# vaultah/replicat

Hardware: AMD Instinct MI355X
Metric: GiB/s chunked, device-resident streams (higher is better)
Workload: dtype u8

## Files before the change

### include/replicat_chunker.h

```cpp
#ifndef REPLICAT_CHUNKER_H
#define REPLICAT_CHUNKER_H

#include <stdint.h>

#ifdef __cplusplus
extern "C" {
#endif

#define RC_OK 0
#define RC_ERR_KEY_LENGTH 1
#define RC_ERR_MIN_GT_MAX 2
#define RC_ERR_BAD_KEY 3
#define RC_ERR_ARGUMENT 10
#define RC_ERR_ALIGN 11
#define RC_ERR_HIP 12
#define RC_ERR_OVERFLOW 13
#define RC_ERR_NO_DEVICE 14
#define RC_ERR_DEVICE_FAULT 15

#define RC_COUNT_OVERFLOW (-1)
#define RC_COUNT_FAULT (-3)

#define RC_OPEN 1u
#define RC_PIPELINED 2u
#define RC_PIPELINE_END 4u

typedef struct rc_chunker rc_chunker;

int rc_version(void);

const char *rc_build_id(void);

const char *rc_last_error(void);

int rc_chunker_create(uint64_t min_length, uint64_t max_length, const uint8_t *key,
                      uint64_t key_len, int device, rc_chunker **out);
void rc_chunker_destroy(rc_chunker *ch);

uint64_t rc_chunker_min_length(const rc_chunker *ch);
uint64_t rc_chunker_max_length(const rc_chunker *ch);

int rc_next_cut(rc_chunker *ch, const uint8_t *buffer, uint64_t size, int final,
                uint64_t *out_cut);

uint64_t rc_cut_capacity(const rc_chunker *ch, uint64_t n, const uint64_t *lens,
                         uint64_t *caps );

int rc_chunk_device(rc_chunker *ch, uint64_t n, const uint8_t *const *d_streams,
                    const uint64_t *lens, const uint64_t *last_piece, uint32_t flags,
                    uint64_t *d_cuts, int64_t *d_counts, void *hip_stream);

int rc_chunker_overlap(rc_chunker *ch, uint32_t reserve_cus);
uint32_t rc_chunker_overlap_cus(const rc_chunker *ch);
uint64_t rc_chunker_pipelined_calls(const rc_chunker *ch);

int rc_chunk_wait(rc_chunker *ch, void *hip_stream);

int rc_stream_create(int device, void **out_stream);
void rc_stream_destroy(void *stream);

int rc_chunk_host(rc_chunker *ch, uint64_t n, const uint8_t *const *streams,
                  const uint64_t *lens, const uint64_t *last_piece, uint32_t flags,
                  uint64_t *cuts, int64_t *counts);

int rc_chunker_check(rc_chunker *ch);

int rc_timing_enable(rc_chunker *ch, int enable);
int rc_timing_read_kernels(rc_chunker *ch, double *tile_ms, double *edge_ms, double *chain_ms,
                           uint64_t *calls);
int rc_timing_read(rc_chunker *ch, double *phase_a_ms, double *phase_b_ms, uint64_t *calls);

int rc_fill_splitmix(uint8_t *d_dst, uint64_t nbytes, uint64_t seed, uint64_t stream,
                     void *hip_stream);
int rc_fill_splitmix_streams(uint8_t *d_dst, uint64_t n, uint64_t nbytes, uint64_t slot,
                             uint64_t seed, uint64_t first_stream, uint64_t stream_step,
                             void *hip_stream);
int rc_fill_splitmix_at(uint8_t *d_dst, uint64_t nbytes, uint64_t seed, uint64_t stream,
                        uint64_t word0, void *hip_stream);

int rc_read_probe(const uint8_t *d_src, uint64_t nbytes, uint32_t *d_out, void *hip_stream);
int rc_chunker_read_probe(rc_chunker *ch, const uint8_t *d_src, uint64_t nbytes, uint32_t *d_out,
                          void *hip_stream);

uint64_t rc_keys_needed(uint64_t max_length, uint64_t L, uint64_t P);

uint64_t rc_host_key(const rc_chunker *ch, uint64_t d);

int rc_tile_records(rc_chunker *ch, uint64_t n, const uint8_t *const *d_streams,
                    const uint64_t *lens, const uint64_t *last_piece, uint64_t *keys,
                    uint64_t *js, uint64_t *gmax, uint64_t *ghot, uint64_t cap,
                    uint64_t *n_tiles);
uint32_t rc_group_hot_threshold(const rc_chunker *ch);
uint64_t rc_tile_keys(void);

int rc_tile_schedule(uint64_t n_tiles, uint32_t waves, uint32_t permille, uint32_t chunk,
                     uint32_t dyn_min, uint32_t *ranges, uint64_t cap, uint64_t *n_units);

int rc_tables_key(const uint8_t *key16, uint64_t n, const uint64_t *ds, uint64_t *out,
                  uint32_t *top16);

#ifdef __cplusplus
}
#endif

#endif
```

### replicat_amd/_lib.py

```python
import ctypes
import os
import threading

HERE = os.path.dirname(os.path.abspath(__file__))
LIB_PATH = os.environ.get('RC_LIB_PATH') or os.path.join(HERE, 'libreplicat_chunker.so')

RC_OK = 0
RC_ERR_KEY_LENGTH = 1
RC_ERR_MIN_GT_MAX = 2
RC_ERR_BAD_KEY = 3
RC_ERR_DIGEST_SIZE = 4
RC_ERR_B2_PARAM = 5
RC_ERR_KEY_SIZE = 6
RC_ERR_NONCE_SIZE = 7
RC_ERR_TAG = 8
RC_ERR_DIGEST_BITS = 9
RC_ERR_ARGUMENT = 10
RC_ERR_ALIGN = 11
RC_ERR_HIP = 12
RC_ERR_OVERFLOW = 13
RC_ERR_NO_DEVICE = 14
RC_ERR_DEVICE_FAULT = 15
RC_ERR_CORRUPT = 16
RC_ERR_INDEX_FULL = 17
RC_ERR_PROBE_BOUND = 18
RC_INDEX_ABSENT, RC_INDEX_EXHAUSTED = -1, -2
RC_GC_REFERENCED, RC_GC_DELETE, RC_GC_TAG_MISMATCH, RC_GC_EXHAUSTED = 0, 1, 2, 3
RC_COUNT_OVERFLOW = -1
RC_COUNT_FAULT = -3
RC_OPEN = 1
RC_PIPELINED = 2
RC_PIPELINE_END = 4
RC_DIGEST_SLOT = 64
RC_HASH_BLAKE2B, RC_HASH_SHA2, RC_HASH_SHA3 = 0, 1, 2
RC_CIPHER_NONE, RC_CIPHER_AES_GCM, RC_CIPHER_CHACHA20_POLY1305 = 0, 1, 2
RC_CHUNK_OK, RC_CHUNK_BAD_TAG, RC_CHUNK_CORRUPT = 0, 1, 2
RC_TABLE_OK, RC_TABLE_BAD_TAG, RC_TABLE_NOT_CANONICAL = 0, 1, 2
RC_PARTS_OK, RC_PARTS_NOT_CANONICAL = 0, 2
RC_PART_FIRST, RC_PART_LAST = 1, 2
RC_SNAPSHOT_PART_WORDS = 8
RC_SNAPSHOT_TEXT_DESC_BYTES = 32

_u64, _i64, _u32, _int, _p = ctypes.c_uint64, ctypes.c_int64, ctypes.c_uint32, ctypes.c_int, ctypes.c_void_p
SIGNATURES = {
    'rc_version': (_int, []),
    'rc_build_id': (ctypes.c_char_p, []),
    'rc_last_error': (ctypes.c_char_p, []),
    'rc_chunker_create': (_int, [_u64, _u64, _p, _u64, _int, ctypes.POINTER(_p)]),
    'rc_chunker_destroy': (None, [_p]),
    'rc_chunker_min_length': (_u64, [_p]),
    'rc_chunker_max_length': (_u64, [_p]),
    'rc_next_cut': (_int, [_p, _p, _u64, _int, ctypes.POINTER(_u64)]),
    'rc_cut_capacity': (_u64, [_p, _u64, _p, _p]),
    'rc_chunk_device': (_int, [_p, _u64, _p, _p, _p, _u32, _p, _p, _p]),
    'rc_chunk_host': (_int, [_p, _u64, _p, _p, _p, _u32, _p, _p]),
    'rc_chunker_overlap': (_int, [_p, _u32]),
    'rc_chunker_overlap_cus': (_u32, [_p]),
    'rc_chunker_pipelined_calls': (_u64, [_p]),
    'rc_chunker_check': (_int, [_p]),
    'rc_chunk_wait': (_int, [_p, _p]),
    'rc_stream_create': (_int, [_int, ctypes.POINTER(_p)]),
    'rc_stream_destroy': (None, [_p]),
    'rc_timing_enable': (_int, [_p, _int]),
    'rc_timing_read': (_int, [_p, ctypes.POINTER(ctypes.c_double), ctypes.POINTER(ctypes.c_double),
                              ctypes.POINTER(_u64)]),
    'rc_timing_read_kernels': (_int, [_p, ctypes.POINTER(ctypes.c_double),
                                      ctypes.POINTER(ctypes.c_double),
                                      ctypes.POINTER(ctypes.c_double), ctypes.POINTER(_u64)]),
    'rc_fill_splitmix': (_int, [_p, _u64, _u64, _u64, _p]),
    'rc_fill_splitmix_at': (_int, [_p, _u64, _u64, _u64, _u64, _p]),
    'rc_fill_splitmix_streams': (_int, [_p, _u64, _u64, _u64, _u64, _u64, _u64, _p]),
    'rc_read_probe': (_int, [_p, _u64, _p, _p]),
    'rc_chunker_read_probe': (_int, [_p, _p, _u64, _p, _p]),
    'rc_keys_needed': (_u64, [_u64, _u64, _u64]),
    'rc_host_key': (_u64, [_p, _u64]),
    'rc_tables_key': (_int, [_p, _u64, _p, _p, _p]),
    'rc_tile_records': (_int, [_p, _u64, _p, _p, _p, _p, _p, _p, _p, _u64, ctypes.POINTER(_u64)]),
    'rc_group_hot_threshold': (_u32, [_p]),
    'rc_tile_keys': (_u64, []),
    'rc_tile_schedule': (_int, [_u64, _u32, _u32, _u32, _u32, _p, _u64, ctypes.POINTER(_u64)]),
    'rc_blake2b_create': (_int, [_u32, _int, ctypes.POINTER(_p)]),
    'rc_blake2b_destroy': (None, [_p]),
    'rc_blake2b_digest_size': (_u32, [_p]),
    'rc_blake2b_device': (_int, [_p, _u64, _p, _p, _p, _p]),
    'rc_blake2b_host': (_int, [_p, _u64, _p, _p, _p]),
    'rc_blake2b_chunks': (_int, [_p, _p, _u64, _p, _p, _p, _p, _p, _p]),
    'rc_chunk_digest_host': (_int, [_p, _p, _u64, _p, _p, _p, _u32, _p, _p, _p]),
    'rc_blake2b_state_init': (_int, [_u32, _p, _u32, _p, _u32, _p, _u32, _p]),
    'rc_blake2b_update_device': (_int, [_p, _u64, _p, _p, _p, _p, _p, _p]),
    'rc_blake2b_timing_enable': (_int, [_p, _int]),
    'rc_blake2b_timing_read': (_int, [_p, ctypes.POINTER(ctypes.c_double), ctypes.POINTER(_u64)]),
    'rc_blake2b_derive_chunks': (_int, [_p, _p, _u64, _p, _p, _p, _p, _u32, _p, _p]),
    'rc_sha2_create': (_int, [_u32, _int, ctypes.POINTER(_p)]),
    'rc_sha3_create': (_int, [_u32, _int, ctypes.POINTER(_p)]),
    'rc_sha2_state_init': (_int, [_u32, _p]),
    'rc_sha3_state_init': (_int, [_u32, _p]),
    'rc_hash_destroy': (None, [_p]),
    'rc_hash_digest_size': (_u32, [_p]),
    'rc_hash_algorithm': (_u32, [_p]),
    'rc_hash_device': (_int, [_p, _u64, _p, _p, _p, _p]),
    'rc_hash_host': (_int, [_p, _u64, _p, _p, _p]),
    'rc_hash_chunks': (_int, [_p, _p, _u64, _p, _p, _p, _p, _p, _p]),
    'rc_hash_update_device': (_int, [_p, _u64, _p, _p, _p, _p, _p, _p]),
    'rc_hash_timing_enable': (_int, [_p, _int]),
    'rc_hash_timing_read': (_int, [_p, ctypes.POINTER(ctypes.c_double), ctypes.POINTER(_u64)]),
    'rc_gcm_create': (_int, [_u32, _u32, _int, ctypes.POINTER(_p)]),
    'rc_gcm_destroy': (None, [_p]),
    'rc_gcm_key_bytes': (_u32, [_p]),
    'rc_gcm_nonce_bytes': (_u32, [_p]),
    'rc_gcm_encrypt_device': (_int, [_p, _u64, _p, _p, _p, _p, _p, _p]),
    'rc_gcm_decrypt_device': (_int, [_p, _u64, _p, _p, _p, _p, _p, _p]),
    'rc_gcm_encrypt_host': (_int, [_p, _u64, _p, _p, _p, _p, _p]),
    'rc_gcm_decrypt_host': (_int, [_p, _u64, _p, _p, _p, _p, _p]),
    'rc_gcm_chunks_layout': (_u64, [_p, _p, _u64, _p, _p]),
    'rc_gcm_encrypt_chunks': (_int, [_p, _p, _u64, _p, _p, _p, _p, _p, _p, _p, _p]),
    'rc_gcm_encrypt_chunks_select': (_int, [_p, _p, _u64, _p, _p, _p, _p, _p, _p, _p, _p, _p, _p, _p]),
    'rc_gcm_timing_enable': (_int, [_p, _int]),
    'rc_gcm_timing_read': (_int, [_p, ctypes.POINTER(ctypes.c_double), ctypes.POINTER(_u64)]),
    'rc_chacha_create': (_int, [_int, ctypes.POINTER(_p)]),
    'rc_chacha_destroy': (None, [_p]),
    'rc_chacha_key_bytes': (_u32, [_p]),
    'rc_chacha_nonce_bytes': (_u32, [_p]),
    'rc_chacha_encrypt_device': (_int, [_p, _u64, _p, _p, _p, _p, _p, _p]),
    'rc_chacha_decrypt_device': (_int, [_p, _u64, _p, _p, _p, _p, _p, _p]),
    'rc_chacha_encrypt_host': (_int, [_p, _u64, _p, _p, _p, _p, _p]),
    'rc_chacha_decrypt_host': (_int, [_p, _u64, _p, _p, _p, _p, _p]),
    'rc_chacha_chunks_layout': (_u64, [_p, _p, _u64, _p, _p]),
    'rc_chacha_encrypt_chunks': (_int, [_p, _p, _u64, _p, _p, _p, _p, _p, _p, _p, _p]),
    'rc_chacha_encrypt_chunks_select': (_int, [_p, _p, _u64, _p, _p, _p, _p, _p, _p, _p, _p, _p, _p, _p]),
    'rc_chacha_timing_enable': (_int, [_p, _int]),
    'rc_chacha_timing_read': (_int, [_p, ctypes.POINTER(ctypes.c_double), ctypes.POINTER(_u64)]),
    'rc_poly1305_host': (_int, [_u64, _p, _p, _p, _p]),
    'rc_restore_create': (_int, [_p, _int, _p, _p, ctypes.POINTER(_p)]),
    'rc_restore_destroy': (None, [_p]),
    'rc_restore_overhead': (_u32, [_p]),
    'rc_restore_verify_device': (_int, [_p, _u64, _p, _p, _p, _p, _p, _p]),
    'rc_restore_verify_host': (_int, [_p, _u64, _p, _p, _p, _p, _p]),
    'rc_restore_timing_enable': (_int, [_p, _int]),
    'rc_restore_timing_read': (_int, [_p, ctypes.POINTER(ctypes.c_double), ctypes.POINTER(_u64)]),
    'rc_index_create': (_int, [_u32, _u64, _int, ctypes.POINTER(_p)]),
    'rc_index_destroy': (None, [_p]),
    'rc_index_name_bytes': (_u32, [_p]),
    'rc_index_used': (_u64, [_p]),
    'rc_index_add_host': (_int, [_p, _u64, _p, ctypes.POINTER(_u64)]),
    'rc_index_resolve_chunks': (_int, [_p, _p, _u64, _p, _p, _p, ctypes.POINTER(_u64), _p, _p, _p]),
    'rc_index_reserve': (_int, [_p, _u64]),
    'rc_index_lookup_device': (_int, [_p, _u64, _p, _p, _p]),
    'rc_index_resolve_names_device': (_int, [_p, _u64, _p, ctypes.POINTER(_u64), _p, _p, _p]),
    'rc_gc_create': (_int, [_u32, _u32, _p, _u32, _u64, _int, ctypes.POINTER(_p)]),
    'rc_gc_destroy': (None, [_p]),
    'rc_gc_name_bytes': (_u32, [_p]),
    'rc_gc_used': (_u64, [_p]),
    'rc_gc_capacity': (_u64, [_p]),
    'rc_gc_reference_host': (_int, [_p, _u64, _p]),
    'rc_gc_reference_device': (_int, [_p, _u64, _p]),
    'rc_gc_sweep_device': (_int, [_p, _u64, _p, _p, _u64, _p, _p, _p, _p]),
    'rc_gc_sweep_host': (_int, [_p, _u64, _p, _p, _p, _p, ctypes.POINTER(_u64)]),
    'rc_gc_unreferenced_host': (_int, [_p, _u64, _p, _p, _p, _p, ctypes.POINTER(_u64)]),
    'rc_gc_timing_enable': (_int, [_p, _int]),
    'rc_gc_timing_read': (_int, [_p, ctypes.POINTER(ctypes.c_double), ctypes.POINTER(ctypes.c_double),
                                 ctypes.POINTER(ctypes.c_double), ctypes.POINTER(_u64)]),
    'rc_snapshot_create': (_int, [_u32, _int, _p, _p, _int, ctypes.POINTER(_p)]),
# ... 129 lines not shown
```

### replicat_amd/csrc/gclmul.h

```cpp
#pragma once
#include <stdint.h>

namespace rc {

#ifndef RC_TILE_ITERS
#define RC_TILE_ITERS 16
#endif
constexpr int kTileIters = RC_TILE_ITERS;
constexpr int kTileKeys = 64 * 4 * kTileIters;
constexpr int kWaveSize = 64;
constexpr int kTileWaves = 16;
constexpr int kChainWaves = 4;
#ifndef RC_TILE_GROUPS
#define RC_TILE_GROUPS 4
#endif
constexpr int kTileGroups = RC_TILE_GROUPS;
constexpr int kGroupKeys = kTileKeys / kTileGroups;

constexpr uint32_t kPfBytes = 131072;
constexpr uint32_t kFullOff = kPfBytes;
constexpr uint32_t kFullBytes = 2 * 4 * 256 * 8;
constexpr uint32_t kTileLdsBytes = kPfBytes + kFullBytes;

struct KeyTables {
// ... 2 lines not shown
    uint32_t pf[4][256];
};

struct StreamDesc {
    const uint8_t *const *ptr;
    const uint64_t *len;
    const uint64_t *last;
    const uint64_t *jneed;
    const uint64_t *tile_base;
    const uint64_t *cut_base;
    const uint64_t *cut_cap;
    const uint64_t *seg_base;
    const uint64_t *scratch_base;
    const uint64_t *xtiles;
};

struct TileRecord {
    uint64_t key;
    uint64_t j;
};

struct GroupRecord {
    uint64_t max;
    uint64_t hot[kTileGroups];
    uint64_t pad;
};
static_assert(kTileGroups % 2 == 0 && sizeof(GroupRecord) % 16 == 0, "group record layout");

__host__ __device__ inline uint32_t group_hot_threshold(uint64_t window) {
    if (window < (uint64_t)kTileKeys) return 0;
    const uint64_t below = (10 * 65536 + window - 1) / window;
    return below >= 65536 ? 0u : (uint32_t)(65536 - below);
}

struct ChainParams {
    uint64_t min_length;
    uint64_t max_length;
    uint64_t window;
    uint64_t max_steps;
    uint64_t seg_bytes;
    uint64_t seg_cap;
    uint64_t ext_steps;
    const GroupRecord *grp;
    uint64_t n_tiles;
    uint32_t open;
    uint32_t lean;
    uint32_t lane;
    uint32_t hot;
    const uint64_t *fault;
    uint64_t epoch;
};

constexpr uint32_t kCtrErrWord = 32, kCtrStampWord = 34, kCtrFaultsWord = 36;
constexpr int64_t kCountFault = -3;

struct TileSched {
    uint32_t permille = 0;
    uint32_t chunk = 3;
    uint32_t dyn_min = 0;
    uint32_t group = 64;
};

__host__ __device__ inline uint64_t splitmix64(uint64_t x) {
    uint64_t z = x + 0x9E3779B97F4A7C15ull;
    z = (z ^ (z >> 30)) * 0xBF58476D1CE4E5B9ull;
    z = (z ^ (z >> 27)) * 0x94D049BB133111EBull;
    return z ^ (z >> 31);
}

}

extern "C" {
int rc_launch_tiles(const rc::KeyTables *d_tables, rc::StreamDesc desc, uint64_t n_streams,
                    uint64_t n_tiles, rc::TileRecord *d_records, rc::GroupRecord *d_grp,
                    uint32_t hot, uint32_t *d_xlist, uint32_t *d_ctr, uint64_t epoch,
                    void *stream, void *mid_event, uint32_t cus, void *edge_stream, void *tiled,
                    rc::TileSched sched);
uint64_t rc_tie_list_words(uint64_t n_tiles);
enum : uint32_t { RC_JOIN_WALK_ONLY = 1, RC_JOIN_REPAIR = 2 };
int rc_launch_chain(const rc::KeyTables *d_tables, rc::StreamDesc desc, uint64_t n_streams,
                    rc::ChainParams prm, uint64_t n_segs, const rc::TileRecord *d_records,
                    uint64_t *d_cuts, int64_t *d_counts, uint64_t *d_scratch,
                    uint64_t *d_seg_counts, bool any_multi, uint32_t join, void *stream);
int rc_launch_fill(uint8_t *d_dst, uint64_t nbytes, uint64_t seed, uint64_t stream_id,
                   uint64_t word0, void *stream);
int rc_launch_fill_streams(uint8_t *d_dst, uint64_t n, uint64_t nbytes, uint64_t slot,
                           uint64_t seed, uint64_t id0, uint64_t id_step, void *stream);
int rc_launch_read_probe(const uint8_t *d_src, uint64_t nbytes, uint32_t *d_out, uint32_t block,
                         rc::TileSched sched, void *stream);
}
```

### replicat_amd/csrc/kernels.hip

```cpp
#include <hip/hip_runtime.h>
#include <stdint.h>

#include "capi_internal.h"
#include "gclmul.h"
#include "diag.h"

using namespace rc;

namespace {

typedef uint32_t u32x4 __attribute__((ext_vector_type(4)));
typedef __attribute__((address_space(1))) const u32x4 gu32x4;
typedef __attribute__((address_space(1))) const uint32_t gu32;

constexpr int kStreamAux = RC_DIAG_STREAM_AUX;

__device__ __forceinline__ __amdgpu_buffer_rsrc_t tile_rsrc(const uint8_t *base,
                                                             uint32_t bytes = 0xffffffffu) {
    return __builtin_amdgcn_make_buffer_rsrc(const_cast<uint8_t *>(base), 0, bytes, 0x00020000);
}
__device__ __forceinline__ u32x4 ring_load(__amdgpu_buffer_rsrc_t r, uint32_t lane_off, int it) {
    return __builtin_amdgcn_raw_buffer_load_b128(r, lane_off, it * 1024, kStreamAux);
}

// ... 1289 lines not shown
                                                      uint64_t *__restrict__ cuts,
                                                      int64_t *__restrict__ counts,
                                                      uint64_t *__restrict__ scratch,
                                                      uint64_t *__restrict__ seg_counts,
                                                      uint64_t *__restrict__ seg_rcount) {
    if (call_faulted(prm)) {
        fault_counts(counts, n_streams);
        return;
    }
    stage_chain_tables(tab);
    const uint32_t *pf = s_chain_lds;
    const uint64_t *full = reinterpret_cast<const uint64_t *>(s_chain_lds + 1024);
    const uint64_t *tl = full, *th = full + 1024;
    const uint32_t lane = lane_id();
    const uint32_t lb_a = (lane & 31) * 4, lb_b = lb_a | 0x10000u;
    const uint64_t q = (uint64_t)blockIdx.x * (blockDim.x >> 6) +
                       __builtin_amdgcn_readfirstlane(threadIdx.x >> 6);
    if (q >= n_segs) return;
    const uint64_t s = find_index(d.seg_base, n_streams + 1, q);
    const uint64_t sb = sload(d.seg_base + s), nseg = sload(d.seg_base + s + 1) - sb;
    const uint64_t i = q - sb;
    ChainStream st = chain_stream(d, s);
    RC_DIAG_ONLY(st.diag = st.diag && i == (nseg > 8 ? 7 : 0);)
    const bool direct = nseg == 1;
    uint64_t *out = direct ? cuts + sload(d.cut_base + s) : scratch + sload(d.scratch_base + s) + i * prm.seg_cap;
    const uint64_t cap = direct ? sload(d.cut_cap + s) : prm.seg_cap;
    const uint64_t seg_end = (i + 1) * prm.seg_bytes;
    const uint64_t steps = prm.max_steps == 0 ? 1 : prm.max_steps;

    uint64_t pos = i * prm.seg_bytes, n = 0, ext = 0;
    bool overflow = false, term = false;
    RecCache<R> cache;
    auto emit = [&](uint64_t c) {
        if (n >= cap) {
            overflow = true;
            return;
        }
        if (lane == 0) out[n] = c;
        ++n;
    };
    for (;;) {
        if (pos >= st.L || n >= steps) {
            term = true;
            break;
        }
        if (!direct && pos >= seg_end && ext++ >= prm.ext_steps) break;
        uint64_t c1 = 0, c2 = 0;
        int kind;
        if constexpr (kLean) {
            static_assert(R == 1, "the lean step works on the one-row cache");
            kind = chain_step_small(tl, th, pf, rec, st, prm, cache, pos, lb_a, lb_b, c1, c2);
        } else {
            kind = chain_step<R>(tl, th, pf, rec, st, prm, cache, pos, lb_a, lb_b, c1, c2);
        }
        if (kind == kStepStop) {
            term = true;
            break;
        }
        emit(c1);
        if (kind == kStepTail2) emit(c2);
        if (kind != kStepCut) {
            term = true;
            break;
        }
        if (overflow) break;
        pos = c1;
    }
    if (lane == 0) {
        if (direct) {
            counts[s] = overflow ? -1 : (int64_t)n;
        } else {
            const uint64_t v = overflow ? ~0ull : (n | (term ? (1ull << 63) : 0));
            seg_counts[q] = v;
            seg_rcount[q] = v;
        }
    }
}

constexpr int kLaneFull = 8;
constexpr int kLaneIters = kTileIters / kTileGroups;

constexpr uint32_t kLaneHotMax = 4;

__device__ __forceinline__ void lane_groups(bool live, const GroupRecord &g, uint32_t te,
                                            uint32_t a, uint32_t b, uint32_t t16, uint32_t hot,
                                            uint64_t (&mk)[kTileGroups], uint32_t &sc) {
    sc = 0;
#pragma unroll
    for (int q = 0; q < kTileGroups; ++q) mk[q] = 0;
    if (!live) return;
    const uint32_t tj0 = te * kTileKeys;
    const uint32_t qa = (a - tj0) / kGroupKeys, qb = (b - tj0) / kGroupKeys;
#pragma unroll
    for (int q = 0; q < kTileGroups; ++q) {
        if ((uint32_t)q < qa || (uint32_t)q > qb) continue;
        if (((uint32_t)(g.max >> (16 * q)) & 0xffffu) < t16) continue;
        const uint32_t nh = (uint32_t)__popcll(g.hot[q]);
        if (t16 < hot || nh > kLaneHotMax || nh == 0) sc |= 1u << q;
        else mk[q] = g.hot[q];
    }
}

__device__ __forceinline__ uint32_t top16_of(uint32_t e_lo_word, uint32_t e_hi_word) {
    return ((e_lo_word & 0xffff0000u) ^ (e_hi_word << 16)) >> 16;
}

template <int U>
__device__ __forceinline__ void scan_range(const uint64_t *tl, const uint64_t *th,
                                           const uint8_t *base, uint64_t a, uint64_t b,
                                           uint64_t &bk, uint64_t &bj) {
    const uint64_t lane = lane_id();
    for (uint64_t r = a; r <= b; r += 64 * U) {
        uint2 w[U];
#pragma unroll
        for (int u = 0; u < U; ++u) {
            const uint64_t j = min(r + 64 * u + lane, b);
            w[u].x = ld_u32(base + 4 * j - 4);
            w[u].y = ld_u32(base + 4 * j);
        }
#pragma unroll
        for (int u = 0; u < U; ++u) {
            const uint64_t j = r + 64 * u + lane;
            if (j <= b) take_best(full_key(tl, th, w[u].x, w[u].y), j, bk, bj);
        }
    }
}

template <int kCtrl>
__device__ __forceinline__ uint32_t qperm32(uint32_t v) {
    return (uint32_t)__builtin_amdgcn_mov_dpp((int)v, kCtrl, 0xf, 0xf, true);
}
template <int kCtrl>
__device__ __forceinline__ uint64_t qperm64(uint64_t v) {
    return (uint64_t)qperm32<kCtrl>((uint32_t)(v >> 32)) << 32 | qperm32<kCtrl>((uint32_t)v);
}
__device__ __forceinline__ void quad_best32(uint64_t &k, uint32_t &j) {
    {
        const uint64_t ko = qperm64<0xB1>(k);
        const uint32_t jo = qperm32<0xB1>(j);
        if (ko > k || (ko == k && jo < j)) k = ko, j = jo;
    }
    {
        const uint64_t ko = qperm64<0x4E>(k);
        const uint32_t jo = qperm32<0x4E>(j);
        if (ko > k || (ko == k && jo < j)) k = ko, j = jo;
    }
}

struct QuadIter {
    u32x4 v;
    uint32_t p;
};

__device__ __forceinline__ QuadIter qi_load(const uint8_t *base, uint32_t j4, uint32_t a,
                                            uint32_t b) {
    QuadIter x = {u32x4{0u, 0u, 0u, 0u}, 0u};
    if (j4 <= b && j4 + 3 >= a) {
        x.v = *as_global_x4(base + 4ull * j4);
        x.p = ld_u32(base + 4ull * j4 - (j4 ? 4 : 0));
    }
    return x;
}

__device__ __forceinline__ void qi_eval(const uint32_t *pf, const uint64_t *tl, const uint64_t *th,
                                        const uint8_t *base, const QuadIter &x, uint32_t j4,
                                        uint32_t a, uint32_t b, uint32_t t16, uint64_t &lk,
                                        uint32_t &lj) {
    if (!(j4 <= b && j4 + 3 >= a)) return;
    const uint32_t wd[5] = {x.p, x.v.x, x.v.y, x.v.z, x.v.w};
    uint32_t e[5];
#pragma unroll
    for (int k = 0; k < 5; ++k) e[k] = pfc_entry(pf, wd[k]);
    bool have = false, tie = false;
    uint32_t ct = 0, cj = 0, clo = 0, chi = 0;
#pragma unroll
    for (int k = 0; k < 4; ++k) {
        const uint32_t j = j4 + k, t = top16_of(e[k], e[k + 1]);
        const bool in = j >= a && j <= b && t >= t16;
        const bool take = in && (!have || t > ct);
        tie = take ? false : (tie || (in && t == ct));
        ct = take ? t : ct;
        cj = take ? j : cj;
        clo = take ? wd[k] : clo;
        chi = take ? wd[k + 1] : chi;
        have = have || in;
    }
    if (have) take_best32(full_key(tl, th, clo, chi), cj, lk, lj);
    if (tie) {
#pragma unroll 1
        for (uint32_t k = 0; k < 4; ++k) {
            const uint32_t j = j4 + k;
            if (j >= a && j <= b)
                take_best32(full_key(tl, th, ld_u32(base + 4ull * j - 4), ld_u32(base + 4ull * j)), j, lk, lj);
        }
    }
}

constexpr int kQuadTasks = 4;

template <int F>
__global__ __launch_bounds__(256) void rc_quad_chain_kernel(const KeyTables *__restrict__ tab,
                                                            StreamDesc d, uint64_t n_streams,
                                                            ChainParams prm,
                                                            const TileRecord *__restrict__ rec,
                                                            uint64_t *__restrict__ cuts,
                                                            int64_t *__restrict__ counts) {
    static_assert(F % 4 == 0 && kLaneIters == 4, "a quad lane per record row and per iteration");
    if (call_faulted(prm)) {
        fault_counts(counts, n_streams);
        return;
    }
    stage_chain_tables(tab);
    const uint32_t *pf = s_chain_lds;
    const uint64_t *full = reinterpret_cast<const uint64_t *>(s_chain_lds + 1024);
    const uint64_t *tl = full, *th = full + 1024;
    const uint32_t lane = lane_id(), q = lane & 3u;
    const uint64_t gid = ((uint64_t)blockIdx.x * blockDim.x + threadIdx.x) >> 2;
    if (gid - (lane >> 2) >= n_streams) return;
    const bool mine = gid < n_streams;
    const uint64_t s = mine ? gid : n_streams - 1;
    const GroupRecord *grp = prm.grp;
    const uint8_t *base = d.ptr[s];
    const uint64_t L = d.len[s], P = d.last[s];
    const uint64_t tb0 = d.tile_base[s], nt = d.tile_base[s + 1] - tb0;
    uint64_t *out = cuts + d.cut_base[s];
    const uint64_t cap = d.cut_cap[s];
    const uint32_t jmax = L >= 8 ? (uint32_t)((L - 4) / 4) : 0u;
    const uint32_t minl = (uint32_t)prm.min_length, maxl = (uint32_t)prm.max_length;
    const uint32_t T = (uint32_t)prm.window;
    auto gtile = [&](bool use, uint32_t t) -> uint64_t { return use && t < nt ? tb0 + t : prm.n_tiles; };

    uint64_t pos = 0, n = 0;
    bool walking = mine && L > 0 && prm.max_steps > 0, overflow = false;
    RC_DIAG_ONLY(const bool diag = gid < 16 && q == 0;)
    for (;;) {
        if (!__any(walking)) break;
        RC_LSTAMP(1);
        const uint64_t rem = L - pos;
        const bool far = rem >= 2ull * maxl;
        const bool argmax = (P >= pos && P - pos >= maxl) || far;
        const uint32_t s4 = (uint32_t)(pos >> 2);
        const uint32_t ja = s4 + 1, jb = min(s4 + T, jmax);
        const bool win = walking && argmax && T > 0 && ja <= jb;
        const uint32_t t_lo = (ja + kTileKeys - 1) / kTileKeys, t_hi = (jb + 1) / kTileKeys;
        const uint32_t nf = win && t_hi > t_lo ? t_hi - t_lo : 0u;
        const uint32_t a0 = ja, b0 = min(jb, t_lo * kTileKeys - 1), te0 = ja / kTileKeys;
        const uint32_t a1 = t_hi * kTileKeys, b1 = jb, te1 = t_hi;
        bool live0 = win && ja < t_lo * kTileKeys;
        bool live1 = win && t_hi >= t_lo && jb >= a1;

        TileRecord fr[F / 4];
#pragma unroll
        for (int i = 0; i < F / 4; ++i) {
            const uint32_t t = 4 * i + q;
            fr[i] = rec[gtile(t < nf, t_lo + t)];
        }
        const TileRecord r0 = rec[gtile(live0, te0)], r1 = rec[gtile(live1, te1)];
        const GroupRecord g0 = grp[gtile(live0, te0)], g1 = grp[gtile(live1, te1)];
        const bool spec = live0;
        const uint32_t lc = (s4 & 255u) >> 2, qc = (s4 & (kTileKeys - 1)) / kGroupKeys;
        const uint32_t jqc = (s4 & ~(uint32_t)(kGroupKeys - 1)) + 4 * lc;
        QuadIter x[kQuadTasks];
        x[0] = qi_load(base, jqc + 256 * q, spec ? a0 : 1u, spec ? b0 : 0u);

        uint64_t bk = 0;
        uint32_t bj = ~0u;
#pragma unroll
        for (int i = 0; i < F / 4; ++i)
            if (4 * (uint32_t)i + q < nf && fr[i].key != 0) take_best32(fr[i].key, (uint32_t)fr[i].j, bk, bj);
        quad_best32(bk, bj);
        if (live0 && edge_settled<false>(r0.key, (uint32_t)r0.j, a0, b0, bk, bj)) live0 = false;
        if (live1 && edge_settled<true>(r1.key, (uint32_t)r1.j, a1, b1, bk, bj)) live1 = false;
        uint32_t sc0, sc1;
        RC_LSTAMP(2);
        uint64_t h[kTileGroups], t[kTileGroups];
        lane_groups(live0, g0, te0, a0, b0, (uint32_t)(bk >> 48), prm.hot, h, sc0);
        lane_groups(live1, g1, te1, a1, b1, (uint32_t)(bk >> 48), prm.hot, t, sc1);
        static_assert(kTileGroups == 4, "the task queue below spells out four groups");
        auto any_task = [&]() { return (h[0] | h[1] | h[2] | h[3] | t[0] | t[1] | t[2] | t[3]) != 0; };
        auto task = [&](uint32_t &jq, uint32_t &a, uint32_t &b) {
            int r = -1;
            uint32_t g = 0, l = 0;
#define RC_POP(M, R, Q)                            \
    if (r < 0 && M) {                              \
        l = (uint32_t)__builtin_ctzll(M);          \
        M &= M - 1;                                \
        r = R;                                     \
        g = Q;                                     \
    }
            RC_POP(h[0], 0, 0) RC_POP(h[1], 0, 1) RC_POP(h[2], 0, 2) RC_POP(h[3], 0, 3)
            RC_POP(t[0], 1, 0) RC_POP(t[1], 1, 1) RC_POP(t[2], 1, 2) RC_POP(t[3], 1, 3)
#undef RC_POP
            a = 1, b = 0;
            if (r < 0) return;
            jq = (r ? te1 : te0) * kTileKeys + g * kGroupKeys + 4 * l;
            a = r ? a1 : a0;
            b = r ? b1 : b0;
        };
        bool first = false;
#define RC_FIRST(Q)                                              \
    if (spec && qc == Q && (h[Q] >> lc & 1u)) {                  \
        h[Q] &= ~(1ull << lc);                                   \
        first = true;                                            \
    }
        RC_FIRST(0) RC_FIRST(1) RC_FIRST(2) RC_FIRST(3)
#undef RC_FIRST
        uint32_t jq[kQuadTasks], ra[kQuadTasks], rb[kQuadTasks];
        jq[0] = jqc, ra[0] = first ? a0 : 1u, rb[0] = first ? b0 : 0u;
        for (;;) {
            if (!__any(first || any_task())) break;
            bool used[kQuadTasks];
#pragma unroll
            for (int k = 0; k < kQuadTasks; ++k) {
                if (!(k == 0 && first)) {
                    task(jq[k], ra[k], rb[k]);
                    x[k] = qi_load(base, jq[k] + 256 * q, ra[k], rb[k]);
                }
                used[k] = __any(ra[k] <= rb[k]);
            }
            const uint32_t t16 = (uint32_t)(bk >> 48);
            uint64_t lk = 0;
            uint32_t lj = ~0u;
#pragma unroll
            for (int k = 0; k < kQuadTasks; ++k)
                if (used[k]) qi_eval(pf, tl, th, base, x[k], jq[k] + 256 * q, ra[k], rb[k], t16, lk, lj);
            quad_best32(lk, lj);
            if (lk != 0) take_best32(lk, lj, bk, bj);
            first = false;
            RC_LSTAMP(3);
        }
        RC_LSTAMP(4);

#pragma unroll 1
        for (int r = 0; r < 2; ++r) {
            const uint32_t sv = r == 0 ? +sc0 : +sc1;
            const uint32_t te = r == 0 ? +te0 : +te1, ra_ = r == 0 ? +a0 : +a1, rb_ = r == 0 ? +b0 : +b1;
            uint32_t sa = 1, sb = 0;
            if (sv) {
                const uint32_t qlo = (uint32_t)__builtin_ctz(sv), qhi = 31u - (uint32_t)__builtin_clz(sv);
                sa = max(ra_, te * kTileKeys + qlo * kGroupKeys);
                sb = min(rb_, te * kTileKeys + (qhi + 1) * kGroupKeys - 1);
            }
            for (uint64_t m = __ballot(q == 0 && sa <= sb); m; m &= m - 1) {
                const int l = __builtin_ctzll(m);
                const uint32_t la = (uint32_t)__builtin_amdgcn_readlane(sa, l);
                const uint32_t lb = (uint32_t)__builtin_amdgcn_readlane(sb, l);
                const uint8_t *lbase = reinterpret_cast<const uint8_t *>(lane_u64((uint64_t)base, l));
                uint64_t ek = 0, ej = ~0ull;
                scan_range<kGroupKeys / 64>(tl, th, lbase, la, lb, ek, ej);
                wave_best(ek, ej);
                if ((lane >> 2) == ((uint32_t)l >> 2) && ek != 0) take_best32(ek, (uint32_t)ej, bk, bj);
                RC_LSTAMP(5);
            }
        }
        RC_LSTAMP(6);

        if (walking) {
            uint64_t c1 = 0, c2 = 0;
            const uint32_t idx = argmax_offset<uint32_t>(bk, bj, s4, minl);
            const int kind = step_cuts(argmax, idx, far, prm.open, pos, rem, minl, maxl, L, c1, c2);
            if (kind != kStepStop) {
                if (n < cap) {
                    if (q == 0) out[n] = c1;
                    ++n;
                } else {
                    overflow = true;
                }
                if (kind == kStepTail2) {
                    if (n < cap) {
                        if (q == 0) out[n] = c2;
                        ++n;
                    } else {
                        overflow = true;
                    }
                }
            }
            if (kind != kStepCut || overflow) walking = false;
            pos = c1;
            if (pos >= L || n >= prm.max_steps) walking = false;
        }
    }
    if (mine && q == 0) counts[s] = overflow ? -1 : (int64_t)n;
}

constexpr uint64_t kNoMerge = ~0ull;
constexpr int64_t kNeedJoin = -2;

constexpr int kRepairSteps = 64;

template <int R>
__global__ __launch_bounds__(256) void rc_merge_kernel(const KeyTables *__restrict__ tab,
                                                       StreamDesc d, uint64_t n_streams,
                                                       ChainParams prm, uint64_t n_segs,
                                                       const TileRecord *__restrict__ rec,
                                                       uint64_t *__restrict__ scratch,
                                                       const uint64_t *__restrict__ seg_counts,
                                                       uint64_t *__restrict__ seg_merge,
                                                       uint64_t *__restrict__ seg_rcount,
                                                       bool repair) {
    if (call_faulted(prm)) return;
    const uint32_t lane = lane_id();
    const uint64_t q = (uint64_t)blockIdx.x * (blockDim.x >> 6) +
                       __builtin_amdgcn_readfirstlane(threadIdx.x >> 6);
    bool active = q < n_segs;
    uint64_t s = 0, k = 0, na = 0, nb = 0, g = 0, ca = ~0ull;
    uint64_t *A = nullptr;
    uint64_t bv = ~0ull, b_last = 0;
    uint64_t result = kNoMerge;
    if (active) {
        s = find_index(d.seg_base, n_streams + 1, q);
        const uint64_t sb = sload(d.seg_base + s), nseg = sload(d.seg_base + s + 1) - sb;
        k = q - sb;
        active = nseg > 1 && k > 0;
    }
    if (active) {
        A = scratch + sload(d.scratch_base + s) + (k - 1) * prm.seg_cap;
        const uint64_t *B = A + prm.seg_cap;
        ca = seg_counts[q - 1];
        const uint64_t cb = seg_counts[q];
        if (ca != ~0ull && cb != ~0ull) {
            na = ca & ~(1ull << 63);
            nb = cb & ~(1ull << 63);
            g = k * prm.seg_bytes;
            const uint64_t a0 = na > 64 ? na - 64 : 0;
            const uint64_t ai = a0 + lane;
            const uint64_t av = ai < na ? A[ai] : 0;
            bv = lane < nb ? B[lane] : ~0ull;
            b_last = lane_u64(bv, 63);
            uint64_t cm = __ballot(ai < na && av >= g);
            const bool whole = a0 == 0 || !(cm & 1ull);
            for (; whole && cm; cm &= cm - 1) {
                const int l = __builtin_ctzll(cm);
                const uint64_t p = lane_u64(av, l);
                if (p == g) {
                    result = (a0 + l + 1) | (0ull << 32);
                    break;
                }
                const uint64_t hit = __ballot(bv == p);
                if (hit) {
                    result = (a0 + l + 1) | ((uint64_t)(__builtin_ctzll(hit) + 1) << 32);
                    break;
                }
                if (nb > 64 && p > b_last) break;
            }
        }
    }
    const bool need = active && result == kNoMerge && ca != ~0ull && (ca >> 63) == 0 && na > 0 &&
                      nb <= 64 && repair;
    if (__syncthreads_or(need)) {
        stage_chain_tables(tab);
        if (need) {
            const uint32_t *pf = s_chain_lds;
            const uint64_t *full = reinterpret_cast<const uint64_t *>(s_chain_lds + 1024);
            const uint64_t *tl = full, *th = full + 1024;
            const uint32_t lb_a = (lane & 31) * 4, lb_b = lb_a | 0x10000u;
            const ChainStream st = chain_stream(d, s);
            RecCache<R> cache;
            uint64_t n = na, pos = A[na - 1];
            const uint64_t b_end = nb ? lane_u64(bv, (int)nb - 1) : 0;
            bool term = false, over = false, past = false;
            for (int step = 0; step < kRepairSteps && result == kNoMerge && !over; ++step) {
                if (pos >= st.L) {
// ... 383 lines not shown
    if (hipDeviceGetAttribute(&cus, hipDeviceAttributeMultiprocessorCount, dev) != hipSuccess ||
        cus <= 0)
        return 256;
    return cus;
}

}

extern "C" {

int rc_launch_tiles(const KeyTables *d_tables, StreamDesc desc, uint64_t n_streams,
                    uint64_t n_tiles, TileRecord *d_records, GroupRecord *d_grp,
                    uint32_t hot, uint32_t *d_xlist, uint32_t *d_ctr, uint64_t epoch,
                    void *stream, void *mid_event, uint32_t tile_cus, void *edge_stream,
                    void *tiled, TileSched sched) {
    hipStream_t st = (hipStream_t)stream;
    hipStream_t est = edge_stream ? (hipStream_t)edge_stream : st;
    auto hand_over = [&]() -> int {
        if (est == st) return 0;
        if ((tiled != mid_event && hipEventRecord((hipEvent_t)tiled, st) != hipSuccess) ||
            hipStreamWaitEvent(est, (hipEvent_t)tiled, 0) != hipSuccess)
            return rc_fail(RC_ERR_HIP, "edge stream hand-over failed");
        return 0;
    };
    if (n_tiles == 0) {
        if (mid_event && hipEventRecord((hipEvent_t)mid_event, st) != hipSuccess)
            return rc_fail(RC_ERR_HIP, "hipEventRecord failed");
        return hand_over();
    }
    const uint64_t waves_per_wg = 1024 / kWaveSize;
    uint64_t grid = (n_tiles + waves_per_wg - 1) / waves_per_wg;
    const uint64_t cus = tile_cus ? (uint64_t)tile_cus : (uint64_t)cu_count();
    if (grid > cus) grid = cus;
    const uint64_t n_waves = grid * waves_per_wg;
    const TileUnits U = tile_units(n_tiles, n_waves, sched);
    uint32_t *d_xcount = d_xlist + n_tiles;
    const bool grp = U.n_groups != 0;
    if (d_grp && grp)
        hipLaunchKernelGGL((rc_tile_kernel<kTileGroups, true>), dim3((unsigned)grid), dim3(1024), 0,
                           st, d_tables, desc, n_streams, U, d_records, d_grp, hot, d_xlist,
                           d_xcount, d_ctr);
    else if (d_grp)
        hipLaunchKernelGGL((rc_tile_kernel<kTileGroups, false>), dim3((unsigned)grid), dim3(1024),
                           0, st, d_tables, desc, n_streams, U, d_records, d_grp, hot, d_xlist,
                           d_xcount, d_ctr);
    else if (grp)
        hipLaunchKernelGGL((rc_tile_kernel<1, true>), dim3((unsigned)grid), dim3(1024), 0, st,
                           d_tables, desc, n_streams, U, d_records, d_grp, hot, d_xlist, d_xcount,
                           d_ctr);
    else
        hipLaunchKernelGGL((rc_tile_kernel<1, false>), dim3((unsigned)grid), dim3(1024), 0, st,
                           d_tables, desc, n_streams, U, d_records, d_grp, hot, d_xlist, d_xcount,
                           d_ctr);
    if (int rc = launch_status("rc_tile_kernel")) return rc;
    if (mid_event && hipEventRecord((hipEvent_t)mid_event, st) != hipSuccess)
        return rc_fail(RC_ERR_HIP, "hipEventRecord failed");
    if (int rc = hand_over()) return rc;
    uint64_t egrid = (U.n_units + 3) / 4;
    if (egrid > 4 * cus) egrid = 4 * cus;
    if (egrid == 0) egrid = 1;
    hipLaunchKernelGGL(rc_edge_kernel, dim3((unsigned)egrid), dim3(256), 0, est, d_tables, desc,
                       n_streams, U, d_records, d_grp, (const uint32_t *)d_xlist,
                       (const uint32_t *)d_xcount, d_ctr, epoch);
    return launch_status("rc_edge_kernel");
}

int rc_tile_schedule(uint64_t n_tiles, uint32_t waves, uint32_t permille, uint32_t chunk,
                     uint32_t dyn_min, uint32_t *ranges, uint64_t cap, uint64_t *n_units) {
    if (!n_units || waves == 0 || n_tiles >= (1ull << 32)) return 1;
    TileSched sched;
    sched.permille = permille;
    sched.chunk = chunk;
    sched.dyn_min = dyn_min;
    const TileUnits U = tile_units(n_tiles, waves, sched);
    *n_units = U.n_units;
    for (uint32_t u = 0; u < U.n_units && u < cap && ranges; ++u) U.range(u, ranges[2 * u], ranges[2 * u + 1]);
    return 0;
}

uint64_t rc_tie_list_words(uint64_t n_tiles) {
    return 2 * n_tiles + n_tiles / kDynChunkMin + 64;
}

int rc_launch_chain(const KeyTables *d_tables, StreamDesc desc, uint64_t n_streams,
                    ChainParams prm, uint64_t n_segs, const TileRecord *d_records,
                    uint64_t *d_cuts, int64_t *d_counts, uint64_t *d_scratch,
                    uint64_t *d_seg_counts, bool any_multi, uint32_t join, void *stream) {
    if (n_streams == 0) return 0;
    hipStream_t st = (hipStream_t)stream;
    if (prm.lane && prm.lean && prm.grp && !any_multi && n_segs == n_streams &&
        prm.max_steps != 0 && prm.window / kTileKeys <= (uint64_t)kLaneFull) {
        const bool narrow = prm.window / kTileKeys <= 4;
        const uint64_t grid = (n_streams + 63) / 64;
        if (narrow)
            hipLaunchKernelGGL(rc_quad_chain_kernel<4>, dim3((unsigned)grid), dim3(256), 0, st,
                               d_tables, desc, n_streams, prm, d_records, d_cuts, d_counts);
        else
            hipLaunchKernelGGL(rc_quad_chain_kernel<kLaneFull>, dim3((unsigned)grid), dim3(256), 0,
                               st, d_tables, desc, n_streams, prm, d_records, d_cuts, d_counts);
        return launch_status("rc_quad_chain_kernel");
    }
    const bool small = prm.window / kTileKeys + 3 <= 64;
    const uint64_t grid = (n_segs + kChainWaves - 1) / kChainWaves;
    uint64_t *seg_merge = d_seg_counts + n_segs, *seg_off = seg_merge + n_segs;
    uint64_t *seg_slice = seg_off + n_segs, *seg_rcount = seg_slice + n_segs;
    if (small && prm.lean)
        hipLaunchKernelGGL((rc_spec_kernel<1, true>), dim3((unsigned)grid),
                           dim3(kChainWaves * kWaveSize), 0, st, d_tables, desc, n_streams, prm,
                           n_segs, d_records, d_cuts, d_counts, d_scratch, d_seg_counts, seg_rcount);
    else if (small)
        hipLaunchKernelGGL((rc_spec_kernel<1, false>), dim3((unsigned)grid),
                           dim3(kChainWaves * kWaveSize), 0, st, d_tables, desc, n_streams, prm,
                           n_segs, d_records, d_cuts, d_counts, d_scratch, d_seg_counts, seg_rcount);
    else
        hipLaunchKernelGGL((rc_spec_kernel<kRecUnroll, false>), dim3((unsigned)grid),
                           dim3(kChainWaves * kWaveSize), 0, st, d_tables, desc, n_streams, prm,
                           n_segs, d_records, d_cuts, d_counts, d_scratch, d_seg_counts, seg_rcount);
    if (int rc = launch_status("rc_spec_kernel")) return rc;
    if (!any_multi) return 0;
    const uint64_t sgrid = (n_segs + 3) / 4, jgrid = (n_streams + kChainWaves - 1) / kChainWaves;
    if (!(join & RC_JOIN_WALK_ONLY)) {
        const bool repair = (join & RC_JOIN_REPAIR) != 0;
        if (small)
            hipLaunchKernelGGL(rc_merge_kernel<1>, dim3((unsigned)sgrid), dim3(256), 0, st,
                               d_tables, desc, n_streams, prm, n_segs, d_records, d_scratch,
                               (const uint64_t *)d_seg_counts, seg_merge, seg_rcount, repair);
        else
            hipLaunchKernelGGL(rc_merge_kernel<kRecUnroll>, dim3((unsigned)sgrid), dim3(256), 0,
                               st, d_tables, desc, n_streams, prm, n_segs, d_records, d_scratch,
                               (const uint64_t *)d_seg_counts, seg_merge, seg_rcount, repair);
        if (int rc = launch_status("rc_merge_kernel")) return rc;
        hipLaunchKernelGGL(rc_scan_kernel, dim3((unsigned)jgrid), dim3(kChainWaves * kWaveSize), 0,
                           st, desc, n_streams, prm, (const uint64_t *)d_seg_counts,
                           (const uint64_t *)seg_merge, (const uint64_t *)seg_rcount, seg_off,
                           seg_slice, d_counts);
        if (int rc = launch_status("rc_scan_kernel")) return rc;
        hipLaunchKernelGGL(rc_copy_kernel, dim3((unsigned)sgrid), dim3(256), 0, st, desc,
                           n_streams, prm, n_segs, (const uint64_t *)d_scratch,
                           (const uint64_t *)seg_off, (const uint64_t *)seg_slice, d_cuts,
                           (const int64_t *)d_counts);
        if (int rc = launch_status("rc_copy_kernel")) return rc;
    } else {
        hipLaunchKernelGGL(rc_mark_kernel, dim3((unsigned)jgrid), dim3(kChainWaves * kWaveSize), 0,
                           st, desc, n_streams, prm, d_counts);
        if (int rc = launch_status("rc_mark_kernel")) return rc;
    }
    if (small)
        hipLaunchKernelGGL(rc_join_kernel<1>, dim3((unsigned)jgrid), dim3(kChainWaves * kWaveSize),
                           0, st, d_tables, desc, n_streams, prm, d_records, d_cuts, d_counts,
                           (const uint64_t *)d_scratch, (const uint64_t *)d_seg_counts);
    else
        hipLaunchKernelGGL(rc_join_kernel<kRecUnroll>, dim3((unsigned)jgrid),
                           dim3(kChainWaves * kWaveSize), 0, st, d_tables, desc, n_streams, prm,
                           d_records, d_cuts, d_counts, (const uint64_t *)d_scratch,
                           (const uint64_t *)d_seg_counts);
    return launch_status("rc_join_kernel");
}

int rc_launch_read_probe(const uint8_t *d_src, uint64_t nbytes, uint32_t *d_out, uint32_t block,
                         TileSched sched, void *stream) {
    const uint64_t n_tiles = nbytes / ((uint64_t)kTileKeys * 4);
    if (n_tiles == 0) return 0;
    uint64_t grid = (n_tiles + 15) / 16;
    const uint64_t cus = (uint64_t)cu_count();
    if (grid > cus) grid = cus;
    const TileUnits U = tile_units(n_tiles, grid * (1024 / kWaveSize), sched);
    if (block == 0 && U.n_units > U.nw &&
        hipMemsetAsync(d_out + 1, 0, sizeof(uint32_t), (hipStream_t)stream) != hipSuccess)
        return rc_fail(RC_ERR_HIP, "hipMemsetAsync failed");
    if (U.n_groups)
        hipLaunchKernelGGL(rc_read_probe_kernel<true>, dim3((unsigned)grid), dim3(1024), 0,
                           (hipStream_t)stream, d_src, n_tiles, d_out, (uint64_t)block, U, d_out + 1);
    else
        hipLaunchKernelGGL(rc_read_probe_kernel<false>, dim3((unsigned)grid), dim3(1024), 0,
                           (hipStream_t)stream, d_src, n_tiles, d_out, (uint64_t)block, U, d_out + 1);
// ... 28 lines not shown
```

Measured before the change: 6896.

## Distribute quad chain group tasks across quad lanes and narrow walk state

Each lane of a quad now owns one tile group: it reads only its own 16-bit max and hot mask, and tasks are popped through a quad-wide min/or permute instead of every lane keeping all four groups' masks. The per-candidate best/tie selection in the quad iterator becomes packed max-based arithmetic, and the walk position and counters shrink to 32-bit. Empty task slots and empty scan rounds are skipped with wave votes, and the scan_range unroll factor is halved. The aim is fewer registers, less redundant record loading and fewer wasted iterations in the chain kernel. The cost is extra cross-lane permutes, and the 32-bit truncation of cut capacity could matter for very large streams.

```diff
diff --git a/include/replicat_chunker.h b/include/replicat_chunker.h
--- a/include/replicat_chunker.h
+++ b/include/replicat_chunker.h
@@ -96,6 +96,8 @@
 int rc_tile_schedule(uint64_t n_tiles, uint32_t waves, uint32_t permille, uint32_t chunk,
                      uint32_t dyn_min, uint32_t *ranges, uint64_t cap, uint64_t *n_units);
 
+uint32_t rc_quad_chain_span(uint64_t min_length, uint64_t max_length);
+
 int rc_tables_key(const uint8_t *key16, uint64_t n, const uint64_t *ds, uint64_t *out,
                   uint32_t *top16);
 
diff --git a/replicat_amd/_lib.py b/replicat_amd/_lib.py
--- a/replicat_amd/_lib.py
+++ b/replicat_amd/_lib.py
@@ -78,6 +78,7 @@
     'rc_tile_records': (_int, [_p, _u64, _p, _p, _p, _p, _p, _p, _p, _u64, ctypes.POINTER(_u64)]),
     'rc_group_hot_threshold': (_u32, [_p]),
     'rc_tile_keys': (_u64, []),
+    'rc_quad_chain_span': (_u32, [_u64, _u64]),
     'rc_tile_schedule': (_int, [_u64, _u32, _u32, _u32, _u32, _p, _u64, ctypes.POINTER(_u64)]),
     'rc_blake2b_create': (_int, [_u32, _int, ctypes.POINTER(_p)]),
     'rc_blake2b_destroy': (None, [_p]),
diff --git a/replicat_amd/csrc/gclmul.h b/replicat_amd/csrc/gclmul.h
--- a/replicat_amd/csrc/gclmul.h
+++ b/replicat_amd/csrc/gclmul.h
@@ -108,6 +108,7 @@
                     rc::ChainParams prm, uint64_t n_segs, const rc::TileRecord *d_records,
                     uint64_t *d_cuts, int64_t *d_counts, uint64_t *d_scratch,
                     uint64_t *d_seg_counts, bool any_multi, uint32_t join, void *stream);
+uint32_t rc_quad_chain_span(uint64_t min_length, uint64_t max_length);
 int rc_launch_fill(uint8_t *d_dst, uint64_t nbytes, uint64_t seed, uint64_t stream_id,
                    uint64_t word0, void *stream);
 int rc_launch_fill_streams(uint8_t *d_dst, uint64_t n, uint64_t nbytes, uint64_t slot,
diff --git a/replicat_amd/csrc/kernels.hip b/replicat_amd/csrc/kernels.hip
--- a/replicat_amd/csrc/kernels.hip
+++ b/replicat_amd/csrc/kernels.hip
@@ -1395,25 +1395,6 @@
 
 constexpr uint32_t kLaneHotMax = 4;
 
-__device__ __forceinline__ void lane_groups(bool live, const GroupRecord &g, uint32_t te,
-                                            uint32_t a, uint32_t b, uint32_t t16, uint32_t hot,
-                                            uint64_t (&mk)[kTileGroups], uint32_t &sc) {
-    sc = 0;
-#pragma unroll
-    for (int q = 0; q < kTileGroups; ++q) mk[q] = 0;
-    if (!live) return;
-    const uint32_t tj0 = te * kTileKeys;
-    const uint32_t qa = (a - tj0) / kGroupKeys, qb = (b - tj0) / kGroupKeys;
-#pragma unroll
-    for (int q = 0; q < kTileGroups; ++q) {
-        if ((uint32_t)q < qa || (uint32_t)q > qb) continue;
-        if (((uint32_t)(g.max >> (16 * q)) & 0xffffu) < t16) continue;
-        const uint32_t nh = (uint32_t)__popcll(g.hot[q]);
-        if (t16 < hot || nh > kLaneHotMax || nh == 0) sc |= 1u << q;
-        else mk[q] = g.hot[q];
-    }
-}
-
 __device__ __forceinline__ uint32_t top16_of(uint32_t e_lo_word, uint32_t e_hi_word) {
     return ((e_lo_word & 0xffff0000u) ^ (e_hi_word << 16)) >> 16;
 }
@@ -1460,6 +1441,48 @@
     }
 }
 
+__device__ __forceinline__ uint32_t quad_or(uint32_t v) {
+    v |= qperm32<0xB1>(v);
+    return v | qperm32<0x4E>(v);
+}
+__device__ __forceinline__ uint32_t quad_min(uint32_t v) {
+    v = min(v, qperm32<0xB1>(v));
+    return min(v, qperm32<0x4E>(v));
+}
+
+__device__ __forceinline__ uint64_t lane_group(bool live, uint32_t q, uint32_t gm, uint64_t gh,
+                                               uint32_t te, uint32_t a, uint32_t b, uint32_t t16,
+                                               uint32_t hot, bool &scan) {
+    const uint32_t tj0 = te * kTileKeys;
+    const uint32_t qa = (a - tj0) / kGroupKeys, qb = (b - tj0) / kGroupKeys;
+    const bool reach = live && q >= qa && q <= qb && gm >= t16;
+    const uint32_t nh = (uint32_t)__popcll(gh);
+    const bool wide = t16 < hot || nh > kLaneHotMax || nh == 0;
+    scan = reach && wide;
+    return reach && !wide ? gh : 0;
+}
+
+struct QuadTasks {
+    uint64_t hm, tm;
+
+    __device__ __forceinline__ bool any() const { return (hm | tm) != 0; }
+    __device__ __forceinline__ bool pop(uint32_t q, uint32_t &g, uint32_t &l) {
+        const uint32_t key = hm != 0 ? q : tm != 0 ? q + kTileGroups : 2u * kTileGroups;
+        g = quad_min(key);
+        const bool mine = key == g && g < 2u * kTileGroups, tail = g >= (uint32_t)kTileGroups;
+        uint64_t m = tail ? tm : hm;
+        uint32_t lm = 0;
+        if (mine) {
+            lm = (uint32_t)__builtin_ctzll(m);
+            m &= m - 1;
+            if (tail) tm = m;
+            else hm = m;
+        }
+        l = quad_or(lm);
+        return g < 2u * kTileGroups;
+    }
+};
+
 struct QuadIter {
     u32x4 v;
     uint32_t p;
@@ -1484,21 +1507,23 @@
     uint32_t e[5];
 #pragma unroll
     for (int k = 0; k < 5; ++k) e[k] = pfc_entry(pf, wd[k]);
-    bool have = false, tie = false;
-    uint32_t ct = 0, cj = 0, clo = 0, chi = 0;
+    uint32_t c[4];
 #pragma unroll
     for (int k = 0; k < 4; ++k) {
         const uint32_t j = j4 + k, t = top16_of(e[k], e[k + 1]);
-        const bool in = j >= a && j <= b && t >= t16;
-        const bool take = in && (!have || t > ct);
-        tie = take ? false : (tie || (in && t == ct));
-        ct = take ? t : ct;
-        cj = take ? j : cj;
-        clo = take ? wd[k] : clo;
-        chi = take ? wd[k + 1] : chi;
-        have = have || in;
-    }
-    if (have) take_best32(full_key(tl, th, clo, chi), cj, lk, lj);
+        c[k] = j >= a && j <= b && t >= t16 ? ((t + 1) << 2 | (uint32_t)(3 - k)) : 0u;
+    }
+    const uint32_t cm = max(max(c[0], c[1]), max(c[2], c[3]));
+    if (cm == 0) return;
+    bool tie = false;
+#pragma unroll
+    for (int k = 0; k < 4; ++k) tie = tie || (c[k] ^ cm) - 1u < 3u;
+    {
+        const bool k1 = !(cm & 1u), k2 = !(cm & 2u);
+        const uint32_t clo = k2 ? (k1 ? wd[3] : wd[2]) : (k1 ? wd[1] : wd[0]);
+        const uint32_t chi = k2 ? (k1 ? wd[4] : wd[3]) : (k1 ? wd[2] : wd[1]);
+        take_best32(full_key(tl, th, clo, chi), j4 + 3u - (cm & 3u), lk, lj);
+    }
     if (tie) {
 #pragma unroll 1
         for (uint32_t k = 0; k < 4; ++k) {
@@ -1535,24 +1560,24 @@
     const GroupRecord *grp = prm.grp;
     const uint8_t *base = d.ptr[s];
     const uint64_t L = d.len[s], P = d.last[s];
-    const uint64_t tb0 = d.tile_base[s], nt = d.tile_base[s + 1] - tb0;
+    const uint64_t tb0 = d.tile_base[s];
+    const uint32_t nt = (uint32_t)(d.tile_base[s + 1] - tb0);
     uint64_t *out = cuts + d.cut_base[s];
-    const uint64_t cap = d.cut_cap[s];
+    const uint32_t cap = (uint32_t)min(d.cut_cap[s], (uint64_t)0xffffffffu);
     const uint32_t jmax = L >= 8 ? (uint32_t)((L - 4) / 4) : 0u;
     const uint32_t minl = (uint32_t)prm.min_length, maxl = (uint32_t)prm.max_length;
     const uint32_t T = (uint32_t)prm.window;
     auto gtile = [&](bool use, uint32_t t) -> uint64_t { return use && t < nt ? tb0 + t : prm.n_tiles; };
 
-    uint64_t pos = 0, n = 0;
+    uint32_t s4 = 0, n = 0;
     bool walking = mine && L > 0 && prm.max_steps > 0, overflow = false;
     RC_DIAG_ONLY(const bool diag = gid < 16 && q == 0;)
     for (;;) {
         if (!__any(walking)) break;
         RC_LSTAMP(1);
-        const uint64_t rem = L - pos;
+        const uint64_t pos = 4ull * s4, rem = L - pos;
         const bool far = rem >= 2ull * maxl;
         const bool argmax = (P >= pos && P - pos >= maxl) || far;
-        const uint32_t s4 = (uint32_t)(pos >> 2);
         const uint32_t ja = s4 + 1, jb = min(s4 + T, jmax);
         const bool win = walking && argmax && T > 0 && ja <= jb;
         const uint32_t t_lo = (ja + kTileKeys - 1) / kTileKeys, t_hi = (jb + 1) / kTileKeys;
@@ -1569,7 +1594,10 @@
             fr[i] = rec[gtile(t < nf, t_lo + t)];
         }
         const TileRecord r0 = rec[gtile(live0, te0)], r1 = rec[gtile(live1, te1)];
-        const GroupRecord g0 = grp[gtile(live0, te0)], g1 = grp[gtile(live1, te1)];
+        const GroupRecord *gr0 = grp + gtile(live0, te0), *gr1 = grp + gtile(live1, te1);
+        const uint32_t gm0 = reinterpret_cast<const uint16_t *>(&gr0->max)[q];
+        const uint32_t gm1 = reinterpret_cast<const uint16_t *>(&gr1->max)[q];
+        const uint64_t gh0 = gr0->hot[q], gh1 = gr1->hot[q];
         const bool spec = live0;
         const uint32_t lc = (s4 & 255u) >> 2, qc = (s4 & (kTileKeys - 1)) / kGroupKeys;
         const uint32_t jqc = (s4 & ~(uint32_t)(kGroupKeys - 1)) + 4 * lc;
@@ -1584,47 +1612,38 @@
         quad_best32(bk, bj);
         if (live0 && edge_settled<false>(r0.key, (uint32_t)r0.j, a0, b0, bk, bj)) live0 = false;
         if (live1 && edge_settled<true>(r1.key, (uint32_t)r1.j, a1, b1, bk, bj)) live1 = false;
-        uint32_t sc0, sc1;
         RC_LSTAMP(2);
-        uint64_t h[kTileGroups], t[kTileGroups];
-        lane_groups(live0, g0, te0, a0, b0, (uint32_t)(bk >> 48), prm.hot, h, sc0);
-        lane_groups(live1, g1, te1, a1, b1, (uint32_t)(bk >> 48), prm.hot, t, sc1);
-        static_assert(kTileGroups == 4, "the task queue below spells out four groups");
-        auto any_task = [&]() { return (h[0] | h[1] | h[2] | h[3] | t[0] | t[1] | t[2] | t[3]) != 0; };
+        QuadTasks tq;
+        bool scan0, scan1;
+        tq.hm = lane_group(live0, q, gm0, gh0, te0, a0, b0, (uint32_t)(bk >> 48), prm.hot, scan0);
+        tq.tm = lane_group(live1, q, gm1, gh1, te1, a1, b1, (uint32_t)(bk >> 48), prm.hot, scan1);
+        const bool first_here = q == qc && (tq.hm >> lc & 1u);
+        if (first_here) tq.hm &= ~(1ull << lc);
+        const uint32_t found = quad_or((scan0 ? 1u << q : 0u) | (scan1 ? 16u << q : 0u) |
+                                       (first_here ? 256u : 0u));
+        const uint32_t sc0 = found & 15u, sc1 = found >> 4 & 15u;
+        bool first = (found & 256u) != 0;
         auto task = [&](uint32_t &jq, uint32_t &a, uint32_t &b) {
-            int r = -1;
             uint32_t g = 0, l = 0;
-#define RC_POP(M, R, Q)                            \
-    if (r < 0 && M) {                              \
-        l = (uint32_t)__builtin_ctzll(M);          \
-        M &= M - 1;                                \
-        r = R;                                     \
-        g = Q;                                     \
-    }
-            RC_POP(h[0], 0, 0) RC_POP(h[1], 0, 1) RC_POP(h[2], 0, 2) RC_POP(h[3], 0, 3)
-            RC_POP(t[0], 1, 0) RC_POP(t[1], 1, 1) RC_POP(t[2], 1, 2) RC_POP(t[3], 1, 3)
-#undef RC_POP
-            a = 1, b = 0;
-            if (r < 0) return;
-            jq = (r ? te1 : te0) * kTileKeys + g * kGroupKeys + 4 * l;
-            a = r ? a1 : a0;
-            b = r ? b1 : b0;
+            const bool have = tq.pop(q, g, l);
+            const bool tail = g >= (uint32_t)kTileGroups;
+            jq = (tail ? te1 : te0) * kTileKeys + (g & (kTileGroups - 1)) * kGroupKeys + 4 * l;
+            if (!have) jq = 4;
+            a = !have ? 1u : tail ? a1 : a0;
+            b = !have ? 0u : tail ? b1 : b0;
         };
-        bool first = false;
-#define RC_FIRST(Q)                                              \
-    if (spec && qc == Q && (h[Q] >> lc & 1u)) {                  \
-        h[Q] &= ~(1ull << lc);                                   \
-        first = true;                                            \
-    }
-        RC_FIRST(0) RC_FIRST(1) RC_FIRST(2) RC_FIRST(3)
-#undef RC_FIRST
         uint32_t jq[kQuadTasks], ra[kQuadTasks], rb[kQuadTasks];
         jq[0] = jqc, ra[0] = first ? a0 : 1u, rb[0] = first ? b0 : 0u;
         for (;;) {
-            if (!__any(first || any_task())) break;
+            if (!__any(first || tq.any())) break;
             bool used[kQuadTasks];
 #pragma unroll
             for (int k = 0; k < kQuadTasks; ++k) {
+                if (k > 0 && !__any(tq.any())) {
+                    jq[k] = 4, ra[k] = 1u, rb[k] = 0u;
+                    used[k] = false;
+                    continue;
+                }
                 if (!(k == 0 && first)) {
                     task(jq[k], ra[k], rb[k]);
                     x[k] = qi_load(base, jq[k] + 256 * q, ra[k], rb[k]);
@@ -1645,7 +1664,7 @@
         RC_LSTAMP(4);
 
 #pragma unroll 1
-        for (int r = 0; r < 2; ++r) {
+        for (int r = 0; r < 2 && __any((sc0 | sc1) != 0); ++r) {
             const uint32_t sv = r == 0 ? +sc0 : +sc1;
             const uint32_t te = r == 0 ? +te0 : +te1, ra_ = r == 0 ? +a0 : +a1, rb_ = r == 0 ? +b0 : +b1;
             uint32_t sa = 1, sb = 0;
@@ -1660,7 +1679,7 @@
                 const uint32_t lb = (uint32_t)__builtin_amdgcn_readlane(sb, l);
                 const uint8_t *lbase = reinterpret_cast<const uint8_t *>(lane_u64((uint64_t)base, l));
                 uint64_t ek = 0, ej = ~0ull;
-                scan_range<kGroupKeys / 64>(tl, th, lbase, la, lb, ek, ej);
+                scan_range<kGroupKeys / 128>(tl, th, lbase, la, lb, ek, ej);
                 wave_best(ek, ej);
                 if ((lane >> 2) == ((uint32_t)l >> 2) && ek != 0) take_best32(ek, (uint32_t)ej, bk, bj);
                 RC_LSTAMP(5);
@@ -1689,8 +1708,8 @@
                 }
             }
             if (kind != kStepCut || overflow) walking = false;
-            pos = c1;
-            if (pos >= L || n >= prm.max_steps) walking = false;
+            if (c1 >= L || n >= prm.max_steps) walking = false;
+            if (walking) s4 = (uint32_t)(c1 >> 2);
         }
     }
     if (mine && q == 0) counts[s] = overflow ? -1 : (int64_t)n;
@@ -2240,6 +2259,17 @@
     return 2 * n_tiles + n_tiles / kDynChunkMin + 64;
 }
 
+static int quad_chain_full(uint64_t window) {
+    const uint64_t f = window / kTileKeys;
+    return f <= 4 ? 4 : f <= (uint64_t)kLaneFull ? kLaneFull : 0;
+}
+
+uint32_t rc_quad_chain_span(uint64_t min_length, uint64_t max_length) {
+    (void)min_length;
+    const int f = quad_chain_full(max_length >= 5 ? (max_length - 1) / 4 : 0);
+    return f ? (uint32_t)f + 2u : 0u;
+}
+
 int rc_launch_chain(const KeyTables *d_tables, StreamDesc desc, uint64_t n_streams,
                     ChainParams prm, uint64_t n_segs, const TileRecord *d_records,
                     uint64_t *d_cuts, int64_t *d_counts, uint64_t *d_scratch,
@@ -2247,8 +2277,8 @@
     if (n_streams == 0) return 0;
     hipStream_t st = (hipStream_t)stream;
     if (prm.lane && prm.lean && prm.grp && !any_multi && n_segs == n_streams &&
-        prm.max_steps != 0 && prm.window / kTileKeys <= (uint64_t)kLaneFull) {
-        const bool narrow = prm.window / kTileKeys <= 4;
+        prm.max_steps != 0 && quad_chain_full(prm.window) != 0) {
+        const bool narrow = quad_chain_full(prm.window) == 4;
         const uint64_t grid = (n_streams + 63) / 64;
         if (narrow)
             hipLaunchKernelGGL(rc_quad_chain_kernel<4>, dim3((unsigned)grid), dim3(256), 0, st,
```

After: 6880. No clear change (-0.2%).
